# gengyuchao/SonicScribe

Hardware: AMD Instinct MI355X
Metric: 20s-segments/sec/node + RTF, GLM-ASR-Nano bf16, batch=32, 1/2/4/8 MI355X (higher is better)
Workload: dtype bf16

## Files before the change

### sonicscribe_amd/csrc/engine.cpp

```cpp
#include "engine_internal.h"

static thread_local std::string g_create_err;

int fail(sonic_engine* e, int code, const char* fmt, ...) {
    char buf[1024];
    va_list ap; va_start(ap, fmt); vsnprintf(buf, sizeof buf, fmt, ap); va_end(ap);
    if (e) e->err = buf; else g_create_err = buf;
    return code;
}

hipError_t h2d(sonic_engine* e, void* dst, const void* src, size_t bytes) {
    hipError_t r = hipMemcpyAsync(dst, src, bytes, hipMemcpyHostToDevice, e->st);
    if (r != hipSuccess) return r;
    return stream_sync(e);
}

hipError_t d2h_async(sonic_engine* e, void* dst, const void* src, size_t bytes) {
    return hipMemcpyAsync(dst, src, bytes, hipMemcpyDeviceToHost, e->st);
}
hipError_t d2h(sonic_engine* e, void* dst, const void* src, size_t bytes) {
    hipError_t r = d2h_async(e, dst, src, bytes);
    return r == hipSuccess ? stream_sync(e) : r;
}
hipError_t stream_sync(sonic_engine* e) {
// ... 272 lines not shown
    for (auto& v : e->gemm_ev) if (hipEventCreate(&v) != hipSuccess) { e->err = "hipEventCreate failed"; return SONIC_ERR_HIP; }
#undef A
    for (auto& v : e->chk_ev) if (hipEventCreateWithFlags(&v, (getenv("SONIC_SPIN_SYNC") ? 0 : hipEventBlockingSync) | hipEventDisableTiming) != hipSuccess) { e->err = "hipEventCreate failed"; return SONIC_ERR_HIP; }
    e->n_samples_h.assign(Bm, 0);
    return SONIC_OK;
}

extern "C" int sonic_create(const sonic_dims* dims, int device_id, int mode, int max_batch, int max_ctx, sonic_engine** out) {
    if (!dims || !out) return fail(nullptr, SONIC_ERR_INVALID, "null argument");
    *out = nullptr;
    if (mode != SONIC_MODE_NATIVE && mode != SONIC_MODE_INT8 && mode != SONIC_MODE_F16 && mode != SONIC_MODE_F32) return fail(nullptr, SONIC_ERR_INVALID, "mode must be either 'native' or 'int8'");
    g_opts = LaunchOpts{};
    TRY(check_dims(*dims, max_batch, max_ctx, mode));
    if (mode == SONIC_MODE_INT8 && (dims->dec_ff > 8192 || dims->enc_d % 128 || dims->enc_ff % 128 || (dims->dec_heads * dims->dec_head_dim) % 128))
        return fail(nullptr, SONIC_ERR_INVALID, "int8 mode: dec_ff must be <= 8192 and every quantised K a multiple of 128");
    int ndev = 0;
    if (hipGetDeviceCount(&ndev) != hipSuccess || ndev <= 0) return fail(nullptr, SONIC_ERR_HIP, "no HIP device available");
    if (device_id < 0 || device_id >= ndev) return fail(nullptr, SONIC_ERR_INVALID, "device %d out of range (%d devices)", device_id, ndev);
    (void)probe_hw_queues(device_id);
    sonic_engine* e = new sonic_engine();
    if (const char* v = getenv("SONIC_KEEP_ROWMAJOR")) e->opt_prefill_rowmajor = atoi(v) >= 2;
    e->d = *dims; e->device = device_id; e->mode = mode; e->Bm = max_batch; e->max_ctx = max_ctx;
    e->i8 = mode == SONIC_MODE_INT8; e->dt = (e->i8 || mode == SONIC_MODE_F16) ? DT_F16 : DT_BF16;
    e->f32 = mode == SONIC_MODE_F32;
    if (e->f32) e->f = new F32State();
    int s = alloc_state(e);
    if (s == SONIC_OK && e->f32) s = f32_alloc(e);
    if (s == SONIC_OK) s = build_constants(e);
    if (s == SONIC_OK && stream_sync(e) != hipSuccess) { e->err = "stream sync failed"; s = SONIC_ERR_HIP; }
    if (s != SONIC_OK) { g_create_err = e->err; sonic_destroy(e); return s; }
    *out = e;
    return SONIC_OK;
}

extern "C" int sonic_slot_create(sonic_engine* parent, sonic_engine** out) {
    if (!parent || !out) return fail(nullptr, SONIC_ERR_INVALID, "null argument");
    *out = nullptr;
    sonic_engine* root = parent->owner ? parent->owner : parent;
    std::lock_guard<std::mutex> lk(root->mu);
    (void)hipGetLastError();
    if (!root->finalized) return fail(nullptr, SONIC_ERR_INVALID, "sonic_slot_create needs an engine whose weights are finalized");
    if (root->f32) return fail(nullptr, SONIC_ERR_UNSUPPORTED, "SONIC_MODE_F32 is a test kind: no slots");
    g_opts = root->opts;
    sonic_engine* e = new sonic_engine();
    e->d = root->d; e->device = root->device; e->mode = root->mode; e->Bm = root->Bm; e->max_ctx = root->max_ctx; e->i8 = root->i8; e->dt = root->dt;
    int s = alloc_state(e);
    if (s == SONIC_OK && stream_sync(e) != hipSuccess) { e->err = "stream sync failed"; s = SONIC_ERR_HIP; }
    if (s != SONIC_OK) { g_create_err = e->err; sonic_destroy(e); return s; }
    e->conv1w = root->conv1w; e->conv2w = root->conv2w; e->conv1b = root->conv1b; e->conv2b = root->conv2b;
    e->enc = root->enc; e->enc_nw = root->enc_nw; e->enc_nb = root->enc_nb; e->gelu_lut = root->gelu_lut;
    e->pj1w = root->pj1w; e->pj2w = root->pj2w; e->pj1b = root->pj1b; e->pj2b = root->pj2b; e->qpj1 = root->qpj1; e->qpj2 = root->qpj2;
    e->embed = root->embed; e->embed_t = root->embed_t; e->dec = root->dec; e->dec_nw = root->dec_nw;
    e->lc = root->lc; e->enc_cs = root->enc_cs; e->dec_cs = root->dec_cs;
    e->opts = root->opts; e->opt_no_graph = root->opt_no_graph; e->opt_no_fused_rope = root->opt_no_fused_rope; e->opt_no_gelu_lut = root->opt_no_gelu_lut;
    e->opt_i8_defer_thr = root->opt_i8_defer_thr; e->opt_i8_no_xq = root->opt_i8_no_xq; e->opt_i8_no_lnq = root->opt_i8_no_lnq; e->opt_i8_no_qkv_fuse = root->opt_i8_no_qkv_fuse;
    e->opt_decode_chunk = root->opt_decode_chunk; e->opt_no_pre_norm = root->opt_no_pre_norm; e->opt_decode_gemv = root->opt_decode_gemv;
    e->weight_bytes = 0; e->finalized = true; e->owner = root;
    root->slots.push_back(e);
    *out = e;
    return SONIC_OK;
}
extern "C" int sonic_engine_info(sonic_engine* e, int32_t* max_batch, int32_t* max_ctx, int32_t* mode, int32_t* device_id, const void** weights_id) {
    if (!e) return SONIC_ERR_INVALID;
    if (max_batch) *max_batch = e->Bm;
    if (max_ctx) *max_ctx = e->max_ctx;
    if (mode) *mode = e->mode;
    if (device_id) *device_id = e->device;
    if (weights_id) *weights_id = e->owner ? (const void*)e->owner : (const void*)e;
    return SONIC_OK;
}
extern "C" int sonic_slot_count(sonic_engine* e) {
    if (!e) return 0;
    sonic_engine* root = e->owner ? e->owner : e;
    std::lock_guard<std::mutex> lk(root->mu);
    return 1 + (int)root->slots.size();
}

extern "C" void sonic_destroy(sonic_engine* e) {
    if (!e) return;
    async_shutdown(e);
    if (e->owner) {
        std::lock_guard<std::mutex> lk(e->owner->mu);
        auto& v = e->owner->slots;
        v.erase(std::remove(v.begin(), v.end(), e), v.end());
    } else {
        std::vector<sonic_engine*> kids;
        { std::lock_guard<std::mutex> lk(e->mu); kids.swap(e->slots); }
        for (sonic_engine* k : kids) { k->owner = nullptr; k->finalized = false; sonic_destroy(k); }
    }
    (void)hipSetDevice(e->device);
    if (e->st) (void)stream_sync(e);
    if (e->splice_ev) {
        sonic_engine* root = e->owner ? e->owner : e;
        std::lock_guard<std::mutex> lk(root->mu);
        if (root != e && root->wait_ev == e->splice_ev) root->wait_pending = false;
        for (sonic_engine* k : root->slots) if (k != e && k->wait_ev == e->splice_ev) k->wait_pending = false;
    }
    for (sonic_ring* r : e->rings) ring_free(r);
    e->rings.clear();
    for (auto& g : e->graphs) (void)hipGraphExecDestroy(g.second);
    for (void* p : e->allocs) (void)hipFree(p);
    if (e->dump) (void)hipFree(e->dump);
    if (e->force_d) (void)hipFree(e->force_d);
    if (e->taps) (void)hipFree(e->taps);
    if (e->feats_f32) (void)hipFree(e->feats_f32);
    if (e->n_active_h) (void)hipHostFree(e->n_active_h);
    for (int i = 0; i < 2; ++i) { if (e->plan_buf[i]) (void)hipHostFree(e->plan_buf[i]); if (e->plan_ev[i]) (void)hipEventDestroy(e->plan_ev[i]); }
// ... 47 lines not shown
```

### sonicscribe_amd/csrc/engine_hooks.cpp

```cpp
#include "engine_internal.h"

template <typename T> __global__ void feats_to_fm_kernel(const float* in, T* out, int n_mels, int n_frames) {
    const int b = blockIdx.y;
    const long e = (long)blockIdx.x * blockDim.x + threadIdx.x;
    if (e >= (long)n_mels * n_frames) return;
    const int t = e / n_mels, m = e % n_mels;
    out[((long)b * (n_frames + 2) + 1 + t) * n_mels + m] = (T)in[((long)b * n_mels + m) * n_frames + t];
}

extern "C" int sonic_logmel(sonic_engine* e, const int16_t* pcm, const int64_t* offsets, int B, float* feats_out, int32_t* mask_out) {
    if (!e) return SONIC_ERR_INVALID;
    ENTER(e);
    TRY(stage_pcm_locked(e, pcm, offsets, B));
    TRY(run_mel(e, B, feats_out != nullptr));
    HIPC(e, stream_sync(e));
    HIPC(e, hipGetLastError());
    const sonic_dims& d = e->d;
    if (feats_out) HIPC(e, d2h(e, feats_out, e->feats_f32, (size_t)B * d.n_mels * d.n_frames * 4));
    if (mask_out)
        for (int b = 0; b < B; ++b) {
            const int v = frames_of(e->n_samples_h[b]);
            for (int t = 0; t < d.n_frames; ++t) mask_out[(size_t)b * d.n_frames + t] = t < v ? 1 : 0;
        }
    return SONIC_OK;
// ... 333 lines not shown
    (void)hipEventRecord(eb, e->st);
    hipError_t r = stream_sync(e);
    float ms = 0; (void)hipEventElapsedTime(&ms, ea, eb);
    (void)hipEventDestroy(ea); (void)hipEventDestroy(eb);
    g_opts = e->opts;
    HIPC(e, r); HIPC(e, hipGetLastError());
    *us_per_launch = ms * 1e3f / iters;
    return SONIC_OK;
}
struct OptRow { const char* key; int sonic_engine::* field; int LaunchOpts::* lfield; bool drop_graphs; int (*clamp)(int); };
#define ENG(m) &sonic_engine::m, nullptr
#define LOP(m) nullptr, &LaunchOpts::m
static const OptRow OPTIONS[] = {
    {"skinny_variant", LOP(skinny_variant), true, nullptr},
    {"gemm_force128", LOP(gemm_force128), false, nullptr},
    {"no_fused_gu", LOP(no_fused_gu), true, nullptr},
    {"no_fused_gu64", LOP(no_fused_gu64), true, nullptr},
    {"gu64_two_pass", LOP(gu64_two_pass), true, nullptr},
    {"gu64_split_norm", LOP(gu64_split_norm), true, nullptr},
    {"ktrace_wave", LOP(ktrace_wave), true, nullptr},
    {"no_skinny768", LOP(no_skinny768), true, nullptr},
    {"no_skinny48", LOP(no_skinny48), true, nullptr},
    {"o64_16rows", LOP(o64_16rows), true, nullptr},
    {"i8_no_lnq", ENG(opt_i8_no_lnq), false, nullptr},
    {"i8_no_qkv_fuse", ENG(opt_i8_no_qkv_fuse), false, nullptr},
    {"i8_dbg", ENG(opt_i8_dbg), true, nullptr},
    {"i8_no_xq", ENG(opt_i8_no_xq), true, nullptr},
    {"gemm_small_eff", LOP(gemm_small_eff), false, nullptr},
    {"gemm128_shallow", LOP(gemm128_shallow), false, nullptr},
    {"no_skinny_i8_wide", LOP(no_skinny_i8_wide), true, nullptr},
    {"gemm256_stagger", LOP(gemm256_stagger), false, nullptr},
    {"flash_variant", LOP(flash_variant), false, nullptr},
    {"flash_enc", LOP(flash_enc), false, nullptr},
    {"gemm256_persist", LOP(gemm256_persist), false, nullptr},
    {"gemm256_persist_cus", LOP(gemm256_persist_cus), false, [](int v) { return v > 0 ? v : 256; }},
    {"gemm256_gm", LOP(gemm256_gm), false, [](int v) { return v > 0 ? v : 8; }},
    {"i8_defer_thr", ENG(opt_i8_defer_thr), false, nullptr},
    {"decode_prefetch", LOP(decode_prefetch), true, nullptr},
    {"decode_attn_occ2", LOP(decode_attn_occ2), true, nullptr},
    {"decode_attn_v1", LOP(decode_attn_v1), true, nullptr},
    {"prefill_taps", ENG(taps_on), false, nullptr},
    {"no_pre_norm", ENG(opt_no_pre_norm), true, nullptr},
    {"decode_gemv", ENG(opt_decode_gemv), true, nullptr},
    {"f32_synth_bf16", ENG(opt_f32_synth_bf16), false, nullptr},
    {"no_graph", ENG(opt_no_graph), false, nullptr},
    {"decode_lookahead", ENG(lookahead), false, [](int v) { return v < 1 ? 1 : (v > CHK_MAX_AHEAD ? CHK_MAX_AHEAD : v); }},
    {"decode_chunk", ENG(opt_decode_chunk), false, [](int v) { return v > 0 ? (v > 64 ? 64 : v) : 1; }},
    {"prefill_rowmajor", ENG(opt_prefill_rowmajor), false, nullptr},
    {"no_rope_tiles", ENG(opt_no_rope_tiles), false, nullptr},
    {"gemm_trace", ENG(opt_gemm_trace), false, nullptr},
    {"gemm_timing", ENG(opt_gemm_timing), false, nullptr},
    {"no_fused_rope", ENG(opt_no_fused_rope), false, nullptr},
    {"no_gelu_lut", ENG(opt_no_gelu_lut), false, nullptr},
};
#undef ENG
#undef LOP
static void drop_graphs(sonic_engine* e) { for (auto& g : e->graphs) (void)hipGraphExecDestroy(g.second); e->graphs.clear(); }
extern "C" int sonic_set_option(sonic_engine* e, const char* key, int value) {
    if (!e || !key) return SONIC_ERR_INVALID;
    std::lock_guard<std::mutex> lk(e->mu);
    for (const OptRow& r : OPTIONS) {
        if (strcmp(key, r.key)) continue;
        const int v = r.clamp ? r.clamp(value) : value;
        if (r.field) e->*r.field = v; else e->opts.*r.lfield = v;
        if (r.drop_graphs) drop_graphs(e);
        return SONIC_OK;
    }
    if (!strcmp(key, "ktrace")) {
        HIPC(e, hipSetDevice(e->device));
        if (value >= 0 && !e->kt) { TRY(dalloc(e, &e->kt, (size_t)8 * KT_SLOT_BLOCKS * 8)); }
        if (e->kt) zero_fill(e, e->kt, (size_t)8 * KT_SLOT_BLOCKS * 8 * 8);
        e->kt_layer = value; drop_graphs(e); return SONIC_OK;
    }
    if (!strcmp(key, "inject_dev_err")) {
        HIPC(e, hipSetDevice(e->device));
        const int v = value ? 1 : 0;
        HIPC(e, hipMemcpyAsync(e->n_active + 1, &v, 4, hipMemcpyHostToDevice, e->st));
        HIPC(e, stream_sync(e));
        return SONIC_OK;
    }
    return fail(e, SONIC_ERR_INVALID, "unknown option %s", key);
}

extern "C" int sonic_debug_read(sonic_engine* e, const char* name, int index, float* out, int64_t n) {
    if (!e || !name || !out) return SONIC_ERR_INVALID;
    ENTER(e);
    const sonic_dims& d = e->d;
    if (e->f32) {
        const float* s32 = nullptr; size_t cap32 = 0;
        if (!strcmp(name, "prefill_tap")) { if (!e->taps) return fail(e, SONIC_ERR_INVALID, "no taps recorded"); s32 = (const float*)e->taps + (size_t)index * e->tok_cap * d.dec_d; cap32 = (size_t)e->tok_cap * d.dec_d; }
        else if (!strcmp(name, "pe")) { s32 = e->f->pe; cap32 = (size_t)e->Bm * e->Ta * d.dec_d; }
        else if (!strcmp(name, "dx")) { s32 = e->f->dx; cap32 = (size_t)e->tok_cap * d.dec_d; }
        else if (!strcmp(name, "enc_x")) { s32 = e->f->ln; cap32 = (size_t)e->Bm * e->T * d.enc_d; }
        else if (!strcmp(name, "h1")) { s32 = e->f->h1; cap32 = (size_t)e->Bm * (d.n_frames + 2) * d.enc_d; }
        else return fail(e, SONIC_ERR_INVALID, "unknown buffer %s", name);
        if (n < 0 || (size_t)n > cap32) return fail(e, SONIC_ERR_INVALID, "read of %lld elements exceeds buffer %s", (long long)n, name);
        HIPC(e, stream_sync(e));
        HIPC(e, d2h(e, out, s32, (size_t)n * 4));
        return SONIC_OK;
    }
    const bf16_t* src = nullptr; size_t cap = 0;
    if (!strcmp(name, "prefill_tap")) { if (!e->taps) return fail(e, SONIC_ERR_INVALID, "no taps recorded"); src = e->taps + (size_t)index * e->tok_cap * d.dec_d; cap = (size_t)e->tok_cap * d.dec_d; }
    else if (!strcmp(name, "pe")) { src = e->pe; cap = (size_t)e->Bm * e->Ta * d.dec_d; }
    else if (!strcmp(name, "dx")) { src = e->dx; cap = (size_t)e->tok_cap * d.dec_d; }
    else if (!strcmp(name, "dqkv")) { src = e->dqkv; cap = (size_t)e->tok_cap * e->qkvN; }
    else if (!strcmp(name, "dq")) { src = e->dq; cap = (size_t)e->tok_cap * e->QD; }
// ... 92 lines not shown
```

### sonicscribe_amd/csrc/engine_internal.h

```cpp
#pragma once
#include <hip/hip_runtime.h>
#include <math.h>
#include <stdarg.h>
#include <stdio.h>
#include <stdlib.h>
#include <string.h>

#include <atomic>
#include <algorithm>
#include <chrono>
#include <condition_variable>
#include <map>
#include <mutex>
#include <string>
#include <thread>
#include <vector>

#include "../../include/sonic_hip.h"
#include "common.h"
#include "kernels.h"

#define T_PAD_ALIGN 64
#define CHK_RING 64
#define DEV_ERR_ACTIVE (-(1 << 23))
// ... 60 lines not shown
    float* dec_nw = nullptr;

    int T = 0, Tp = 0, Ta = 0, hd_e = 0, qkvN = 0, QD = 0, KD = 0, tok_cap = 0, out_cap = 0;
    long slabN = 0;

    int16_t* pcm = nullptr; int* n_samples_d = nullptr; std::vector<int> n_samples_h; int W = 0;
    float* logspec = nullptr; int* segmax = nullptr; bf16_t* feats_fm = nullptr; float* feats_f32 = nullptr;
    LogmelConst lc{};
    bf16_t *h1 = nullptr, *x = nullptr, *ln = nullptr, *qk = nullptr, *vt = nullptr, *att = nullptr, *ff = nullptr, *ph = nullptr, *pe = nullptr;
    float* enc_cs = nullptr;
    bf16_t *dx = nullptr, *dhn = nullptr, *dqkv = nullptr, *dq = nullptr, *datt = nullptr, *dact = nullptr;
    bf16_t *Kc = nullptr, *Vc = nullptr, *Vts = nullptr;
    float* dec_cs = nullptr;
    float *slab = nullptr, *lslab = nullptr, *ssq = nullptr;
    float* slab2 = nullptr;
    bf16_t *sx = nullptr, *shn = nullptr, *sq = nullptr, *satt = nullptr, *sact = nullptr;
    bf16_t* sx2 = nullptr;
    int *kv_len = nullptr, *tok_pos = nullptr, *n_new = nullptr, *finished = nullptr, *max_new_d = nullptr, *n_active = nullptr;
    int *out_ids = nullptr, *step_ctr = nullptr, *seq_iota = nullptr;
    int *src = nullptr, *tok_seq = nullptr, *tok_pos_pf = nullptr, *q_off = nullptr, *q_len = nullptr, *last_row = nullptr;
    float* dump = nullptr; size_t dump_cap = 0; int dump_steps = 0;
    bf16_t* taps = nullptr; int taps_on = 0; int last_ntok = 0;
    int* n_active_h = nullptr;
    int R = 0, max_steps = 0, greedy_calls = 0, steps_run = 0; bool run_logits = false;
    int* force_d = nullptr; int force_ld = 0, force_R = 0;
    std::vector<int> last_qlen, last_maxnew;
    std::map<std::pair<int, int>, hipGraphExec_t> graphs;
    hipEvent_t chk_ev[CHK_RING]{};
    bool run_starved = false;
    int lookahead = 1;
    int* plan_h = nullptr; size_t plan_cap = 0;
    int* plan_buf[2] = {nullptr, nullptr}; hipEvent_t plan_ev[2] = {nullptr, nullptr}; bool plan_busy[2] = {false, false}; int plan_idx = 0;

    sonic_engine* owner = nullptr;
    std::vector<sonic_engine*> slots;
    std::mutex rings_mu;

    bool svc_on = false;
    int64_t svc_launched = 0, svc_checked = 0;
    int64_t svc_dry = 0;
    int svc_calm = 0;
    int* svc_h = nullptr;
    int svc_fin[64]{}, svc_nn[64]{}, svc_active = 0; int64_t svc_seq = 0;
    hipEvent_t sync_ev = nullptr;
    hipStream_t st_io = nullptr;
    hipEvent_t xfer_ev = nullptr, splice_ev = nullptr, wait_ev = nullptr; bool wait_pending = false;

    struct AsyncJob { std::vector<int32_t> req_win, prompt_ids, max_new; std::vector<int64_t> prompt_off; int R = 0; bool has_rw = false; int want_logits = 0; } a_job;
    std::thread a_thread; std::mutex a_mu; std::condition_variable a_cv;
    bool a_started = false, a_pending = false, a_running = false, a_done = false, a_stop = false; int a_status = 0;

    LaunchOpts opts;
    int opt_no_graph = 0, opt_gemm_timing = 0, opt_no_fused_rope = 0, opt_no_gelu_lut = 0, opt_gemm_trace = 0, opt_no_rope_tiles = 0, opt_prefill_rowmajor = 0;
    double host_launch_ms = 0, host_wait_ms = 0; int host_launches = 0;
    int step_launches_per_layer = 0;
    int opt_f32_synth_bf16 = 0;
    int opt_decode_gemv = 0;
    int opt_no_pre_norm = 0;
    int opt_decode_chunk = 2;
    long long* kt = nullptr; int kt_layer = -1;
    int* ring_peak = nullptr;
    std::vector<struct sonic_ring*> rings;

    hipEvent_t ev[5]{};
    std::vector<hipEvent_t> gemm_ev;
    int gemm_ev_used = 0;
    sonic_timings tim{};
};

struct QGroup { const int* gmap; int gdiv; int G; };
struct QkvVt { bf16_t* Vt; int n_split, seg_T, vt_ld; long vt_seg_stride; };

struct HostPlan {
    std::vector<int> src, tok_seq, tok_pos, q_off, q_len, last_row, max_new;
    int n_tok = 0, max_p = 0, max_steps = 0;
};

#define HIPC(e, call)                                                                                      \
    do {                                                                                                   \
        hipError_t _r = (call);                                                                            \
        if (_r != hipSuccess) {                                                                            \
            const bool oom = (_r == hipErrorOutOfMemory);                                                  \
            return fail(e, oom ? SONIC_ERR_OOM : SONIC_ERR_HIP, "%s%s failed: %s (%s:%d)",                 \
                        oom ? "HIP out of memory: " : "", #call, hipGetErrorString(_r), __FILE__, __LINE__); \
        }                                                                                                  \
    } while (0)

#define TRY(x) do { int _s = (x); if (_s != SONIC_OK) return _s; } while (0)
#define ENTER(e) std::lock_guard<std::mutex> lk((e)->mu); (void)hipGetLastError(); HIPC(e, hipSetDevice((e)->device)); g_opts = (e)->opts

int fail(sonic_engine* e, int code, const char* fmt, ...);
hipError_t stream_sync(sonic_engine* e);
hipError_t h2d(sonic_engine* e, void* dst, const void* src, size_t bytes);
hipError_t d2h_async(sonic_engine* e, void* dst, const void* src, size_t bytes);
hipError_t d2h(sonic_engine* e, void* dst, const void* src, size_t bytes);
void zero_fill(sonic_engine* e, void* q, size_t bytes);
template <typename Tt> static int dalloc(sonic_engine* e, Tt** p, size_t n, bool zero = true) {
    void* q = nullptr;
    const size_t bytes = ((n ? n : 1) * sizeof(Tt) + 3) / 4 * 4;
    HIPC(e, hipMalloc(&q, bytes));
    e->allocs.push_back(q); e->alloc_bytes += (int64_t)bytes;
    if (zero) zero_fill(e, q, bytes);
    *p = (Tt*)q;
    return SONIC_OK;
}

void gemm(sonic_engine* e, int epi, const bf16_t* A, long lda, const bf16_t* W, const float* bias, bf16_t* C, long ldc,
          int M, int N, int K, const bf16_t* R = nullptr, long ldr = 0, int w_tiled = 0, int gu8 = 0);
bool qlinear(sonic_engine* e, int epi, const bf16_t* X, long ldx, const bf16_t* w16, const QW& q, const float* bias, bf16_t* C, long ldc,
             int M, int N, int K, const bf16_t* R, long ldr, const QGroup& grp, const float* rope_cs = nullptr, int rope_T = 0, int rope_ncols = 0,
             bool prequant = false, const QkvVt* vt = nullptr);
int run_mel(sonic_engine* e, int W, bool want_f32);
int run_encoder(sonic_engine* e, int W, float* enc_layers_out, float* enc_out_host, int n_groups);
int keep_rows(const sonic_dims& d, int n_valid_frames);
int frames_of(int n_samples);
void skinny(sonic_engine* e, const bf16_t* X, long ldx, const bf16_t* W, float* P, int M, int N, int K, int* ks_out, long long* kt = nullptr);
GreedyArgs greedy_args(sonic_engine* e, int R, bool dump);
void decode_step_i8(sonic_engine* e, int R, bool dump);
int run_to_first_token(sonic_engine* e, const int32_t* req_win, int R, const int32_t* prompt_ids, const int64_t* prompt_off,
                       const int32_t* max_new, bool want_logits);
int chunk_graph(sonic_engine* e, int R, int n, hipGraphExec_t* out, bool svc = false);
int run_decode_steps(sonic_engine* e, int n_steps, int* done_out);
int run_all(sonic_engine* e, const int32_t* req_win, int R, const int32_t* prompt_ids, const int64_t* prompt_off,
            const int32_t* max_new, bool want_logits);

int f32_alloc(sonic_engine* e);
int f32_finalize(sonic_engine* e);
int f32_run_encoder(sonic_engine* e, int W, float* enc_layers_out, float* enc_out_host);
GreedyArgs f32_greedy_args(sonic_engine* e, int R, bool dump);
int f32_run_prefill(sonic_engine* e, int R, const HostPlan& hp);
void decode_step_f32(sonic_engine* e, int R, bool dump);

int stage_pcm_locked(sonic_engine* e, const int16_t* pcm, const int64_t* offsets, int W);
void ring_free(sonic_ring* r);
void async_shutdown(sonic_engine* e);
int fetch_locked(sonic_engine* e, int32_t* out_ids, int out_ld, int32_t* out_len, float* step_logits);
```

### sonicscribe_amd/csrc/engine_stages.cpp

```cpp
#include "engine_internal.h"

void gemm(sonic_engine* e, int epi, const bf16_t* A, long lda, const bf16_t* W, const float* bias, bf16_t* C, long ldc,
          int M, int N, int K, const bf16_t* R, long ldr, int w_tiled, int gu8) {
    GemmArgs a{};
    a.A = A; a.lda = lda; a.W = W; a.C = C; a.ldc = ldc; a.bias = bias; a.R = R; a.ldr = ldr; a.M = M; a.N = N; a.K = K; a.batch = 1; a.dt = e->dt;
    a.w_tiled = w_tiled; a.gu8 = gu8;
    a.gelu_lut = e->opt_no_gelu_lut ? nullptr : e->gelu_lut;
    launch_gemm(a, epi, e->st);
}
static QuantActArgs make_qa(sonic_engine* e, const bf16_t* X, long ldx, int M, int K, const QGroup& grp) {
    QuantActArgs qa{};
    qa.X = X; qa.ld = ldx; qa.M = M; qa.K = K; qa.gmap = grp.gmap; qa.gdiv = grp.gdiv; qa.G = grp.G; qa.flags = e->q_flags;
    qa.q = e->qa; qa.sca = e->q_sca; qa.oc_cnt = e->q_oc_cnt; qa.oc_list = e->q_oc_list; qa.oc_ld = e->q_kmax;
    return qa;
}
static bool layernorm_q(sonic_engine* e, const bf16_t* x, const float* w, const float* b, bf16_t* y, int M, int d, float eps, const QGroup& grp) {
    if (e->i8 && !e->opt_i8_no_lnq) {
        const QuantActArgs qa = make_qa(e, y, d, M, d, grp);
        launch_quant_act_begin(qa, e->st);
        launch_layernorm(x, w, b, y, M, d, eps, e->st, e->dt, &qa);
        return true;
    }
    launch_layernorm(x, w, b, y, M, d, eps, e->st, e->dt);
    return false;
}
static bool rmsnorm_q(sonic_engine* e, const bf16_t* x, const float* w, bf16_t* y, int M, int d, float eps, const QGroup& grp) {
    if (e->i8 && !e->opt_i8_no_lnq) {
        const QuantActArgs qa = make_qa(e, y, d, M, d, grp);
        launch_quant_act_begin(qa, e->st);
        launch_rmsnorm(x, w, y, M, d, eps, nullptr, e->st, e->dt, &qa);
        return true;
    }
    launch_rmsnorm(x, w, y, M, d, eps, nullptr, e->st, e->dt);
    return false;
}
bool qlinear(sonic_engine* e, int epi, const bf16_t* X, long ldx, const bf16_t* w16, const QW& q, const float* bias, bf16_t* C, long ldc,
             int M, int N, int K, const bf16_t* R, long ldr, const QGroup& grp, const float* rope_cs, int rope_T, int rope_ncols,
             bool prequant, const QkvVt* vt) {
    if (!e->i8 || !(q.cb || q.cbt)) { gemm(e, epi, X, ldx, w16, bias, C, ldc, M, N, K, R, ldr); return false; }
    const QuantActArgs qa = make_qa(e, X, ldx, M, K, grp);
    if (prequant) launch_quant_act_finish(qa, e->st);
    else launch_quant_act(qa, e->st);
    GemmArgs a{};
    a.A = (const bf16_t*)e->qa; a.lda = K; a.W = (const bf16_t*)q.cb; a.C = C; a.ldc = ldc; a.bias = bias; a.R = R; a.ldr = ldr; a.M = M; a.N = N; a.K = K; a.batch = 1; a.dt = DT_F16;
    if (q.cbt && (!e->opt_prefill_rowmajor || !q.cb_rowmajor_kept)) { a.W = (const bf16_t*)q.cbt; a.w_tiled = 1; }
    a.q.sca = e->q_sca; a.q.scb = q.scb; a.q.x16 = X; a.q.ldx16 = ldx; a.q.oc_cnt = e->q_oc_cnt; a.q.oc_list = e->q_oc_list; a.q.oc_ld = e->q_kmax;
    a.q.row_group = grp.gmap; a.q.group_div = grp.gdiv;
    bool fuse = false;
    if (vt && rope_cs && !e->opt_i8_no_qkv_fuse && !g_opts.gemm_force128) {
        GemmArgs t = a; t.Vt = vt->Vt; t.n_split = vt->n_split; t.seg_T = vt->seg_T; t.vt_ld = vt->vt_ld; t.vt_seg_stride = vt->vt_seg_stride;
        if (gemm256_eligible(t, EPI_QKV_VT)) { a = t; a.rope_cs = rope_cs; a.rope_T = rope_T; a.rope_ncols = rope_ncols; epi = EPI_QKV_VT; fuse = true; }
    }
    const bool defer = epi == EPI_BIAS_RESID && e->defer_tmp && e->opt_i8_defer_thr >= 0 && (size_t)M * ldc <= e->defer_cap;
    if (defer) { a.q.defer_out = e->defer_tmp; a.q.defer_thr = e->opt_i8_defer_thr; }
    launch_gemm(a, epi, e->st);
    if (defer) launch_i8_outlier_side(a, e->st);
    return fuse;
}

int run_mel(sonic_engine* e, int W, bool want_f32) {
    const sonic_dims& d = e->d;
    if (want_f32 && !e->feats_f32) {
        HIPC(e, hipMalloc((void**)&e->feats_f32, (size_t)e->Bm * d.n_mels * d.n_frames * 4));
    }
    int mx = 0; for (int i = 0; i < W; ++i) mx = e->n_samples_h[i] > mx ? e->n_samples_h[i] : mx;
    launch_logmel(e->pcm, (long)d.n_frames * 160, e->n_samples_d, mx, e->lc, e->logspec, e->segmax, W, d.n_frames, d.n_mels,
                  e->feats_fm, want_f32 ? e->feats_f32 : nullptr, e->st, e->dt);
    return SONIC_OK;
}

int run_encoder(sonic_engine* e, int W, float* enc_layers_out, float* enc_out_host, int n_groups) {
    const sonic_dims& d = e->d;
    const int C = d.enc_d, T = e->T, M = W * T, H = d.enc_heads, dt = e->dt;
    const QGroup grp{e->win_req, T, n_groups}, grp_p{e->win_req, e->Ta, n_groups};
    {
        GemmArgs a{};
        a.A = e->feats_fm; a.lda = d.n_mels; a.W = e->conv1w; a.bias = e->conv1b; a.C = e->h1 + C; a.ldc = C; a.dt = dt;
        a.M = d.n_frames; a.N = C; a.K = 3 * d.n_mels; a.batch = W;
        a.strideA = (long)(d.n_frames + 2) * d.n_mels; a.strideC = (long)(d.n_frames + 2) * C;
        launch_gemm(a, EPI_BIAS_GELU, e->st);
        GemmArgs b{};
        b.A = e->h1; b.lda = 2L * C; b.W = e->conv2w; b.bias = e->conv2b; b.C = e->x; b.ldc = C; b.dt = dt;
        b.M = T; b.N = C; b.K = 3 * C; b.batch = W; b.strideA = (long)(d.n_frames + 2) * C; b.strideC = (long)T * C;
        launch_gemm(b, EPI_BIAS_GELU, e->st);
    }
    float* tap = nullptr;
    if (enc_layers_out || enc_out_host) HIPC(e, hipMalloc((void**)&tap, (size_t)M * C * 4));
    e->gemm_ev_used = 0;
    for (int l = 0; l < d.enc_layers; ++l) {
        const EncLayerW& L = e->enc[l];
        const bool pq1 = layernorm_q(e, e->x, L.ln1w, L.ln1b, e->ln, M, C, d.enc_ln_eps, grp);
        const bool tev = e->opt_gemm_timing && (size_t)(8 * l + 7) < e->gemm_ev.size();
        auto mark = [&](int i) { if (tev) (void)hipEventRecord(e->gemm_ev[8 * l + i], e->st); };
        FlashArgs f{};
        f.dt = dt; f.T = T; f.Hq = H; f.Hkv = H; f.scale = 1.0f / sqrtf((float)e->hd_e); f.Vt = e->vt; f.vt_ld = e->Tp; f.O = e->att; f.o_ld = C;
        f.k_head_stride = e->hd_e; f.vt_seq_stride = (long)C * e->Tp; f.vt_head_stride = (long)e->hd_e * e->Tp;
        if (e->i8) {
            mark(0);
            const bool can_fuse = e->hd_e == 64 && d.enc_rotary_dim == 32 && !e->opt_no_fused_rope;
            const QkvVt vt{e->vt, 2 * C, T, e->Tp, (long)C * e->Tp};
            const bool fused = qlinear(e, EPI_BIAS, e->ln, C, nullptr, L.qqkv, L.bqkv, e->qkv_rm, 3L * C, M, 3 * C, C, nullptr, 0, grp,
                                       can_fuse ? e->enc_cs : nullptr, T, 2 * C, pq1, &vt);
            mark(1);
            if (!fused) {
                launch_rope_enc(e->qkv_rm, 3L * C, M, T, 2 * H, e->hd_e, d.enc_rotary_dim, e->enc_cs, e->st, dt);
                launch_transpose_v(e->qkv_rm, 3L * C, 2 * C, e->vt, W, T, C, e->Tp, (long)C * e->Tp, e->st);
            }
            f.Q = e->qkv_rm; f.q_ld = 3L * C; f.K = e->qkv_rm + C; f.k_ld = 3L * C;
            f.q_seq_stride = (long)T * 3 * C; f.k_seq_stride = (long)T * 3 * C;
        } else {
            GemmArgs a{};
            a.A = e->ln; a.lda = C; a.W = L.wqkv; a.bias = L.bqkv; a.C = e->qk; a.ldc = 2L * C; a.M = M; a.N = 3 * C; a.K = C; a.batch = 1; a.dt = dt;
            a.Vt = e->vt; a.n_split = 2 * C; a.seg_T = T; a.vt_ld = e->Tp; a.vt_seg_stride = (long)C * e->Tp;
            const bool roped = e->hd_e == 64 && d.enc_rotary_dim == 32 && !e->opt_no_fused_rope && !g_opts.gemm_force128 && gemm256_eligible(a, EPI_QKV_VT);
            if (roped) { a.rope_cs = e->enc_cs; a.rope_T = T; a.rope_ncols = 2 * C; }
            mark(0);
            launch_gemm(a, EPI_QKV_VT, e->st);
            mark(1);
            if (!roped) launch_rope_enc(e->qk, 2L * C, M, T, 2 * H, e->hd_e, d.enc_rotary_dim, e->enc_cs, e->st, dt);
            f.Q = e->qk; f.q_ld = 2L * C; f.K = e->qk + C; f.k_ld = 2L * C;
            f.q_seq_stride = (long)T * 2 * C; f.k_seq_stride = (long)T * 2 * C;
        }
        launch_flash(f, 64, false, W, T, e->st);
        mark(2);
        qlinear(e, EPI_BIAS_RESID, e->att, C, L.wo, L.qo, L.bo, e->x, C, M, C, C, e->x, C, grp);
        mark(3);
        const bool pq2 = layernorm_q(e, e->x, L.ln2w, L.ln2b, e->ln, M, C, d.enc_ln_eps, grp);
        mark(4);
        qlinear(e, EPI_BIAS_GELU, e->ln, C, L.w1, L.q1, L.b1, e->ff, d.enc_ff, M, d.enc_ff, C, nullptr, 0, grp, nullptr, 0, 0, pq2);
        mark(5);
        if (tev) e->gemm_ev_used = l + 1;
        mark(6);
        qlinear(e, EPI_BIAS_RESID, e->ff, d.enc_ff, L.w2, L.q2, L.b2, e->x, C, M, C, d.enc_ff, e->x, C, grp);
        mark(7);
        if (enc_layers_out) {
            launch_bf16_to_f32(e->x, tap, (long)M * C, e->st, dt);
            HIPC(e, stream_sync(e));
            for (int b = 0; b < W; ++b)
                HIPC(e, d2h(e, enc_layers_out + ((size_t)b * d.enc_layers + l) * T * C, tap + (size_t)b * T * C, (size_t)T * C * 4));
        }
    }
    launch_layernorm(e->x, e->enc_nw, e->enc_nb, e->ln, M, C, d.enc_ln_eps, e->st, dt);
    if (enc_out_host) {
        launch_bf16_to_f32(e->ln, tap, (long)M * C, e->st, dt);
        HIPC(e, stream_sync(e));
        HIPC(e, d2h(e, enc_out_host, tap, (size_t)M * C * 4));
    }
    if (tap) (void)hipFree(tap);
    const int Mp = W * e->Ta, PI = C * d.merge, PM = 2 * d.dec_d;
    qlinear(e, EPI_BIAS_GELU, e->ln, PI, e->pj1w, e->qpj1, e->pj1b, e->ph, PM, Mp, PM, PI, nullptr, 0, grp_p);
    qlinear(e, EPI_BIAS, e->ph, PM, e->pj2w, e->qpj2, e->pj2b, e->pe, d.dec_d, Mp, d.dec_d, PM, nullptr, 0, grp_p);
    return SONIC_OK;
}

static int floordiv(int a, int b) { int q = a / b; return (a % b != 0 && ((a < 0) != (b < 0))) ? q - 1 : q; }
int keep_rows(const sonic_dims& d, int n_valid_frames) {
    int L = n_valid_frames;
    L = floordiv(L + 2 - 2 - 1, 1) + 1;
    L = floordiv(L + 2 - 2 - 1, 2) + 1;
    const int k = floordiv(L - d.merge, d.merge) + 1;
    const int Ta = d.enc_T / d.merge;
    return k < 0 ? 0 : (k > Ta ? Ta : k);
}
int frames_of(int n_samples) { return n_samples > 0 ? (n_samples + 159) / 160 : 0; }

static long long* kt_slot(sonic_engine* e, int l, int slot) { return (e->kt && l == e->kt_layer) ? e->kt + (long)slot * KT_SLOT_BLOCKS * 8 : nullptr; }
void skinny(sonic_engine* e, const bf16_t* X, long ldx, const bf16_t* W, float* P, int M, int N, int K, int* ks_out, long long* kt) {
    SkinnyArgs a{}; a.kt = kt;
    a.X = X; a.ldx = ldx; a.W = W; a.P = P; a.M = M; a.N = N; a.K = K; a.ksplit = skinny_pick_ksplit(N, K); a.dt = e->dt;
    if (ks_out) *ks_out = a.ksplit;
    launch_skinny(a, e->st);
}
static int skinny_i8_xq(sonic_engine* e, const bf16_t* X16, const float* amax, const int8_t* Wt, float* P, int M, int N, int K) {
    SkinnyArgs a{};
    a.X = X16; a.ldx = K; a.W = (const bf16_t*)Wt; a.P = P; a.M = M; a.N = N; a.K = K; a.ksplit = skinny_pick_ksplit_i8(N, K); a.i8 = 1; a.x_amax = amax;
    launch_skinny(a, e->st);
    return a.ksplit;
}
static int skinny_i8(sonic_engine* e, const int8_t* Xq, const int8_t* Wt, float* P, int M, int N, int K) {
    SkinnyArgs a{};
    a.X = (const bf16_t*)Xq; a.ldx = K; a.W = (const bf16_t*)Wt; a.P = P; a.M = M; a.N = N; a.K = K; a.ksplit = skinny_pick_ksplit_i8(N, K); a.i8 = 1;
    launch_skinny(a, e->st);
    return a.ksplit;
}

GreedyArgs greedy_args(sonic_engine* e, int R, bool dump) {
    const sonic_dims& d = e->d;
    GreedyArgs g{};
    g.logits = e->lslab; g.ksplit = skinny_pick_ksplit(d.vocab, d.dec_d); g.mpad = ((R + 15) / 16) * 16; g.V = d.vocab; g.B = R; g.table = e->embed; g.x = e->sx; g.d = d.dec_d;
    g.out_ids = e->out_ids; g.out_ld = e->out_cap; g.n_new = e->n_new; g.finished = e->finished; g.kv_len = e->kv_len; g.tok_pos = e->tok_pos;
    g.max_new = e->max_new_d; g.n_active = e->n_active; g.dev_err = e->n_active + 1; g.n_eos = d.n_eos; g.pad_id = d.n_eos > 0 ? d.eos[0] : 0;
    for (int i = 0; i < d.n_eos; ++i) g.eos[i] = d.eos[i];
    g.logits_dump = dump ? e->dump : nullptr; g.dump_stride_step = (long)R * d.vocab; g.step_counter = dump ? e->step_ctr : nullptr;
    g.norm_w = e->dec.empty() ? nullptr : e->dec[0].ln1; g.norm_eps = d.dec_rms_eps; g.y = e->dec.empty() ? nullptr : e->shn;
    g.force_ids = e->force_d; g.force_ld = e->force_ld;
    g.dt = e->dt;
    if (e->i8) g.qo = QuantOut{e->hn_q, d.dec_d, e->sca_hn, e->oc_hn, e->ol_hn, d.dec_d, e->ov_hn};
    return g;
}

static void decode_step(sonic_engine* e, int R, bool dump) {
    if (e->f32) { decode_step_f32(e, R, dump); return; }
// ... 256 lines not shown
    if (e->wait_pending) {
        HIPC(e, hipStreamWaitEvent(e->st, e->wait_ev, 0));
        e->wait_pending = false;
    }
    HostPlan hp;
    TRY(plan_requests(e, req_win, R, prompt_ids, prompt_off, max_new, hp));
    {
        const int i = e->plan_idx ^ 1;
        if (e->plan_busy[i]) { HIPC(e, hipEventSynchronize(e->plan_ev[i])); e->plan_busy[i] = false; }
        e->plan_idx = i; e->plan_h = e->plan_buf[i];
    }
    if (e->force_d && (e->force_R != R || e->force_ld < hp.max_steps))
        return fail(e, SONIC_ERR_INVALID, "forced ids are [%d][%d] but the run has %d requests / %d steps", e->force_R, e->force_ld, R, hp.max_steps);
    e->R = R; e->max_steps = hp.max_steps; e->last_qlen = hp.q_len; e->last_maxnew = hp.max_new;
    if (want_logits) {
        const size_t need_n = (size_t)hp.max_steps * R * d.vocab;
        if (need_n > e->dump_cap) {
            if (e->dump) (void)hipFree(e->dump);
            e->dump = nullptr; e->dump_cap = 0;
            HIPC(e, hipMalloc((void**)&e->dump, need_n * 4));
            e->dump_cap = need_n;
        }
        e->dump_steps = hp.max_steps;
    } else e->dump_steps = 0;
    e->run_logits = want_logits;

    if (e->f32) {
        (void)hipEventRecord(e->ev[0], e->st);
        TRY(run_mel(e, e->W, true));
        (void)hipEventRecord(e->ev[1], e->st);
        TRY(f32_run_encoder(e, e->W, nullptr, nullptr));
        (void)hipEventRecord(e->ev[2], e->st);
        TRY(f32_run_prefill(e, R, hp));
        launch_greedy(f32_greedy_args(e, R, want_logits), e->st);
        (void)hipEventRecord(e->ev[3], e->st);
        e->steps_run = 0; e->greedy_calls = 1;
        return SONIC_OK;
    }
    (void)hipEventRecord(e->ev[0], e->st);
    TRY(run_mel(e, e->W, false));
    (void)hipEventRecord(e->ev[1], e->st);
    {
        std::vector<int> wr(64, 0);
        for (int r = 0; r < R; ++r) {
            const int w0 = req_win ? req_win[r] : r, w1 = req_win ? req_win[r + 1] : r + 1;
            for (int w = w0; w < w1 && w < 64; ++w) wr[w] = r;
        }
        if (e->i8) {
            int* h = e->plan_h + e->plan_cap - 64;
            memcpy(h, wr.data(), 64 * 4);
            HIPC(e, hipMemcpyAsync(e->win_req, h, 64 * 4, hipMemcpyHostToDevice, e->st));
        }
    }
    TRY(run_encoder(e, e->W, nullptr, nullptr, R));
    (void)hipEventRecord(e->ev[2], e->st);
    TRY(run_prefill(e, R, hp));
    launch_greedy(greedy_args(e, R, want_logits), e->st);
    (void)hipEventRecord(e->ev[3], e->st);
    e->steps_run = 0;
    e->greedy_calls = 1;
    return SONIC_OK;
}

int chunk_graph(sonic_engine* e, int R, int n, hipGraphExec_t* out, bool svc) {
    const std::pair<int, int> key{R + (svc ? 4096 : 0), n};
    auto it = e->graphs.find(key);
    if (it != e->graphs.end()) { *out = it->second; return SONIC_OK; }
    hipGraph_t g = nullptr; hipGraphExec_t gx = nullptr;
    HIPC(e, hipStreamBeginCapture(e->st, hipStreamCaptureModeThreadLocal));
    e->cap_svc = svc;
    for (int i = 0; i < n; ++i) decode_step(e, R, false);
    e->cap_svc = false;
    HIPC(e, hipStreamEndCapture(e->st, &g));
    hipError_t r = hipGraphInstantiate(&gx, g, nullptr, nullptr, 0);
    (void)hipGraphDestroy(g);
    HIPC(e, r);
    e->graphs[key] = gx;
    *out = gx;
    return SONIC_OK;
}

int run_decode_steps(sonic_engine* e, int n_steps, int* done_out) {
    const int R = e->R, left = e->max_steps - 1 - e->steps_run;
    if (n_steps > left) n_steps = left;
    const bool want_logits = e->run_logits;
    const bool use_graph = !want_logits && !e->opt_no_graph && !e->force_d && !e->f32;
    const int C = e->opt_decode_chunk > 0 ? e->opt_decode_chunk : 1;
    int done = 0;
    int launched = 0, checked = 0, last_grow = 0;
    bool all_stopped = false, starved = false, dev_err = false;
    typedef std::chrono::steady_clock clk;
    auto ms_since = [](clk::time_point t0) { return std::chrono::duration<double, std::milli>(clk::now() - t0).count(); };
    auto read_check = [&](bool block) -> int {
        const int i = checked % CHK_RING;
        if (!block) { const hipError_t q = hipEventQuery(e->chk_ev[i]); if (q == hipErrorNotReady) { (void)hipGetLastError(); return 0; } if (q != hipSuccess) return -1; }
        else { const auto t_w = clk::now(); if (hipEventSynchronize(e->chk_ev[i]) != hipSuccess) return -1; e->host_wait_ms += ms_since(t_w); }
        if (e->n_active_h[i] <= 0) all_stopped = true;
        if (e->n_active_h[i] < DEV_ERR_ACTIVE) dev_err = true;
        ++checked;
        return 1;
    };
    while (done < n_steps && !all_stopped) {
        const int n = n_steps - done < C ? n_steps - done : C;
        if (launched > 0 && hipEventQuery(e->chk_ev[(launched - 1) % CHK_RING]) == hipSuccess) {
            if (launched - last_grow > e->lookahead && e->lookahead < CHK_MAX_AHEAD) {
                e->lookahead = e->lookahead * 2 < CHK_MAX_AHEAD ? e->lookahead * 2 : CHK_MAX_AHEAD;
                last_grow = launched;
// ... 70 lines not shown
```

Before: 172.3.

## Prune encoder last-layer rows past the longest valid segment in the batch

Computes the largest number of adapter rows any window in the batch keeps and, when it is below the full encoder length, runs only those rows through the last encoder layer's post-attention path, the final layernorm and the projector GEMMs. The full attention in that layer still runs, and the dropped tail rows are ones the decoder never reads. This cuts GEMM work for batches of short segments. It only applies in the non-int8 path, adds a new strided batched GEMM path, and can be turned off with the no_enc_prune option.

```diff
diff --git a/sonicscribe_amd/csrc/engine.cpp b/sonicscribe_amd/csrc/engine.cpp
--- a/sonicscribe_amd/csrc/engine.cpp
+++ b/sonicscribe_amd/csrc/engine.cpp
@@ -348,7 +348,7 @@
     e->pj1w = root->pj1w; e->pj2w = root->pj2w; e->pj1b = root->pj1b; e->pj2b = root->pj2b; e->qpj1 = root->qpj1; e->qpj2 = root->qpj2;
     e->embed = root->embed; e->embed_t = root->embed_t; e->dec = root->dec; e->dec_nw = root->dec_nw;
     e->lc = root->lc; e->enc_cs = root->enc_cs; e->dec_cs = root->dec_cs;
-    e->opts = root->opts; e->opt_no_graph = root->opt_no_graph; e->opt_no_fused_rope = root->opt_no_fused_rope; e->opt_no_gelu_lut = root->opt_no_gelu_lut;
+    e->opts = root->opts; e->opt_no_graph = root->opt_no_graph; e->opt_no_fused_rope = root->opt_no_fused_rope; e->opt_no_gelu_lut = root->opt_no_gelu_lut; e->opt_no_enc_prune = root->opt_no_enc_prune;
     e->opt_i8_defer_thr = root->opt_i8_defer_thr; e->opt_i8_no_xq = root->opt_i8_no_xq; e->opt_i8_no_lnq = root->opt_i8_no_lnq; e->opt_i8_no_qkv_fuse = root->opt_i8_no_qkv_fuse;
     e->opt_decode_chunk = root->opt_decode_chunk; e->opt_no_pre_norm = root->opt_no_pre_norm; e->opt_decode_gemv = root->opt_decode_gemv;
     e->weight_bytes = 0; e->finalized = true; e->owner = root;
diff --git a/sonicscribe_amd/csrc/engine_hooks.cpp b/sonicscribe_amd/csrc/engine_hooks.cpp
--- a/sonicscribe_amd/csrc/engine_hooks.cpp
+++ b/sonicscribe_amd/csrc/engine_hooks.cpp
@@ -409,6 +409,7 @@
     {"gemm_timing", ENG(opt_gemm_timing), false, nullptr},
     {"no_fused_rope", ENG(opt_no_fused_rope), false, nullptr},
     {"no_gelu_lut", ENG(opt_no_gelu_lut), false, nullptr},
+    {"no_enc_prune", ENG(opt_no_enc_prune), false, nullptr},
 };
 #undef ENG
 #undef LOP
diff --git a/sonicscribe_amd/csrc/engine_internal.h b/sonicscribe_amd/csrc/engine_internal.h
--- a/sonicscribe_amd/csrc/engine_internal.h
+++ b/sonicscribe_amd/csrc/engine_internal.h
@@ -136,6 +136,7 @@
 
     LaunchOpts opts;
     int opt_no_graph = 0, opt_gemm_timing = 0, opt_no_fused_rope = 0, opt_no_gelu_lut = 0, opt_gemm_trace = 0, opt_no_rope_tiles = 0, opt_prefill_rowmajor = 0;
+    int opt_no_enc_prune = 0;
     double host_launch_ms = 0, host_wait_ms = 0; int host_launches = 0;
     int step_launches_per_layer = 0;
     int opt_f32_synth_bf16 = 0;
@@ -195,7 +196,7 @@
              int M, int N, int K, const bf16_t* R, long ldr, const QGroup& grp, const float* rope_cs = nullptr, int rope_T = 0, int rope_ncols = 0,
              bool prequant = false, const QkvVt* vt = nullptr);
 int run_mel(sonic_engine* e, int W, bool want_f32);
-int run_encoder(sonic_engine* e, int W, float* enc_layers_out, float* enc_out_host, int n_groups);
+int run_encoder(sonic_engine* e, int W, float* enc_layers_out, float* enc_out_host, int n_groups, bool prune = false);
 int keep_rows(const sonic_dims& d, int n_valid_frames);
 int frames_of(int n_samples);
 void skinny(sonic_engine* e, const bf16_t* X, long ldx, const bf16_t* W, float* P, int M, int N, int K, int* ks_out, long long* kt = nullptr);
diff --git a/sonicscribe_amd/csrc/engine_stages.cpp b/sonicscribe_amd/csrc/engine_stages.cpp
--- a/sonicscribe_amd/csrc/engine_stages.cpp
+++ b/sonicscribe_amd/csrc/engine_stages.cpp
@@ -69,10 +69,24 @@
     return SONIC_OK;
 }
 
-int run_encoder(sonic_engine* e, int W, float* enc_layers_out, float* enc_out_host, int n_groups) {
+int run_encoder(sonic_engine* e, int W, float* enc_layers_out, float* enc_out_host, int n_groups, bool prune) {
     const sonic_dims& d = e->d;
     const int C = d.enc_d, T = e->T, M = W * T, H = d.enc_heads, dt = e->dt;
     const QGroup grp{e->win_req, T, n_groups}, grp_p{e->win_req, e->Ta, n_groups};
+    int Tk = T;
+    if (prune && !e->i8 && !e->opt_no_enc_prune && !enc_layers_out && !enc_out_host && d.enc_layers > 0 && (int)e->n_samples_h.size() >= W) {
+        int mx = 1;
+        for (int w = 0; w < W; ++w) { const int k = keep_rows(d, frames_of(e->n_samples_h[w])); mx = k > mx ? k : mx; }
+        if (mx * d.merge < T) Tk = mx * d.merge;
+    }
+    auto gemm_win = [&](int epi, const bf16_t* A, long lda, long sA, const bf16_t* Wt, const float* bias, bf16_t* Cc, long ldc, long sC, int Mw, int N, int K,
+                        const bf16_t* R, long ldr, long sR) {
+        GemmArgs a{};
+        a.A = A; a.lda = lda; a.W = Wt; a.C = Cc; a.ldc = ldc; a.bias = bias; a.R = R; a.ldr = ldr; a.M = Mw; a.N = N; a.K = K; a.dt = dt;
+        a.batch = W; a.strideA = sA; a.strideC = sC; a.strideR = sR;
+        a.gelu_lut = e->opt_no_gelu_lut ? nullptr : e->gelu_lut;
+        launch_gemm(a, epi, e->st);
+    };
     {
         GemmArgs a{};
         a.A = e->feats_fm; a.lda = d.n_mels; a.W = e->conv1w; a.bias = e->conv1b; a.C = e->h1 + C; a.ldc = C; a.dt = dt;
@@ -121,6 +135,22 @@
             f.Q = e->qk; f.q_ld = 2L * C; f.K = e->qk + C; f.k_ld = 2L * C;
             f.q_seq_stride = (long)T * 2 * C; f.k_seq_stride = (long)T * 2 * C;
         }
+        if (Tk < T && l == d.enc_layers - 1) {
+            const int Mc = W * Tk;
+            launch_flash(f, 64, false, W, Tk, e->st);
+            mark(2);
+            gemm_win(EPI_BIAS_RESID, e->att, C, (long)T * C, L.wo, L.bo, e->ln, C, (long)Tk * C, Tk, C, C, e->x, C, (long)T * C);
+            mark(3);
+            launch_layernorm(e->ln, L.ln2w, L.ln2b, e->att, Mc, C, d.enc_ln_eps, e->st, dt);
+            mark(4);
+            gemm(e, EPI_BIAS_GELU, e->att, C, L.w1, L.b1, e->ff, d.enc_ff, Mc, d.enc_ff, C);
+            mark(5);
+            if (tev) e->gemm_ev_used = l + 1;
+            mark(6);
+            gemm(e, EPI_BIAS_RESID, e->ff, d.enc_ff, L.w2, L.b2, e->x, C, Mc, C, d.enc_ff, e->ln, C);
+            mark(7);
+            break;
+        }
         launch_flash(f, 64, false, W, T, e->st);
         mark(2);
         qlinear(e, EPI_BIAS_RESID, e->att, C, L.wo, L.qo, L.bo, e->x, C, M, C, C, e->x, C, grp);
@@ -140,7 +170,7 @@
                 HIPC(e, d2h(e, enc_layers_out + ((size_t)b * d.enc_layers + l) * T * C, tap + (size_t)b * T * C, (size_t)T * C * 4));
         }
     }
-    launch_layernorm(e->x, e->enc_nw, e->enc_nb, e->ln, M, C, d.enc_ln_eps, e->st, dt);
+    launch_layernorm(e->x, e->enc_nw, e->enc_nb, e->ln, W * Tk, C, d.enc_ln_eps, e->st, dt);
     if (enc_out_host) {
         launch_bf16_to_f32(e->ln, tap, (long)M * C, e->st, dt);
         HIPC(e, stream_sync(e));
@@ -148,6 +178,12 @@
     }
     if (tap) (void)hipFree(tap);
     const int Mp = W * e->Ta, PI = C * d.merge, PM = 2 * d.dec_d;
+    if (Tk < T) {
+        const int tk = Tk / d.merge;
+        gemm(e, EPI_BIAS_GELU, e->ln, PI, e->pj1w, e->pj1b, e->ph, PM, W * tk, PM, PI);
+        gemm_win(EPI_BIAS, e->ph, PM, (long)tk * PM, e->pj2w, e->pj2b, e->pe, d.dec_d, (long)e->Ta * d.dec_d, tk, d.dec_d, PM, nullptr, 0, 0);
+        return SONIC_OK;
+    }
     qlinear(e, EPI_BIAS_GELU, e->ln, PI, e->pj1w, e->qpj1, e->pj1b, e->ph, PM, Mp, PM, PI, nullptr, 0, grp_p);
     qlinear(e, EPI_BIAS, e->ph, PM, e->pj2w, e->qpj2, e->pj2b, e->pe, d.dec_d, Mp, d.dec_d, PM, nullptr, 0, grp_p);
     return SONIC_OK;
@@ -510,7 +546,7 @@
             HIPC(e, hipMemcpyAsync(e->win_req, h, 64 * 4, hipMemcpyHostToDevice, e->st));
         }
     }
-    TRY(run_encoder(e, e->W, nullptr, nullptr, R));
+    TRY(run_encoder(e, e->W, nullptr, nullptr, R, true));
     (void)hipEventRecord(e->ev[2], e->st);
     TRY(run_prefill(e, R, hp));
     launch_greedy(greedy_args(e, R, want_logits), e->st);
```

Measured after the change: 171.6. No clear change (-0.4%).
